# Rikorose/DeepFilterNet

Hardware: AMD Instinct MI355X
Metric: 48 kHz audio frames/sec (hop=480), DeepFilterNet3 enhance() (higher is better)
Workload: dtype f32 (storage and accumulation; GRU projections / recurrences, the fused DF-encoder convolutions and the pointwise halves of the ERB separable convolutions as fp16-split MFMAs: x = hi + lo in f16, hi*hi + hi*lo + lo*hi on v_mfma_f32_16x16x32_f16, ~2^-21 relative; see exact_fp32_ms_per_step); 1 GPU; DeepFilterNet3 (recalled shipped shape, conv_ch=64) enhance(pad=True), batch=256 clips x 10 s @48 kHz per GPU, 1002 STFT frames per clip; batch_per_gpu=256, global_batch=256, parallelism=clips sharded over 1 GPU(s); no collective, inputs_resident_in_hbm=True

## Files before the change

deepfilternet_amd/csrc/dfx_nn_kernels.h:

```cpp
#pragma once

#include "dfx_common.h"

#include <type_traits>

#define DFX_ACT_NONE 0
#define DFX_ACT_RELU 1
#define DFX_ACT_TANH 2
#define DFX_ACT_SIGMOID 3

static __device__ __forceinline__ float dfx_sigmoid(float x) { return 1.f / (1.f + expf(-x)); }
static __device__ __forceinline__ float dfx_act(float v, int act) {
    if (act == DFX_ACT_RELU) return fmaxf(v, 0.f);
    if (act == DFX_ACT_TANH) return tanhf(v);
    if (act == DFX_ACT_SIGMOID) return dfx_sigmoid(v);
    return v;
}

static __device__ __forceinline__ float dfx_row256_scale_split(const float4 (&raw)[16], dfx_h8 (&xh)[8], dfx_h8 (&xl)[8]) {
    float mx = 0.f;
#pragma unroll
    for (int i = 0; i < 16; ++i) mx = fmaxf(mx, fmaxf(fmaxf(fabsf(raw[i].x), fabsf(raw[i].y)), fmaxf(fabsf(raw[i].z), fabsf(raw[i].w))));
    mx = fmaxf(mx, __shfl_xor(mx, 16));
    mx = fmaxf(mx, __shfl_xor(mx, 32));
// ... 3940 lines not shown
    dfx_h8 *wl = reinterpret_cast<dfx_h8 *>(smraw);
    uint16_t *h16 = reinterpret_cast<uint16_t *>(smraw + DFX_GH_SMEM_W);
    float *h32 = reinterpret_cast<float *>(smraw + DFX_GH_SMEM_W);
    static_assert((size_t)2 * DFX_GH_ROWS * DFX_GH_HROW32 * 4 <= (size_t)2 * 2 * DFX_GH_ROWS * DFX_GH_HROW * 2, "the fp32 copy of h fits where the f16 copies live");
    constexpr size_t HB_KSTEP = X32 ? 32 * 4 : 32 * 2, HB_LO = X32 ? 16 : (size_t)DFX_GH_ROWS * HROW * 2;
    const int tid = threadIdx.x, lane = tid & 63, wave = tid >> 6, q = lane >> 4, jl = lane & 15;
    const int64_t b0 = grp * DFX_GH_ROWS;
    const bool valid = b0 + jl < A.B;
    const int64_t brow = valid ? b0 + jl : A.B - 1;
    const dfx_h8 *wg = A.whf + lane;
#define DFX_GH_GIDX(f) (((((size_t)wave * NS + DFX_GH_POS_S(f)) * 8 + DFX_GH_POS_KC(f)) * 3 + DFX_GH_POS_GATE(f)) * 2 * 64)
    dfx_h8 wr[FR][2];
    dfx_static_for<0, NF>([&](auto fc) {
        constexpr int f = decltype(fc)::value;
        if constexpr (SC.cls[f] == 0) {
            wr[SC.idx[f]][0] = wg[DFX_GH_GIDX(f)];
            wr[SC.idx[f]][1] = wg[DFX_GH_GIDX(f) + 64];
            if constexpr (DFX_GH_PIN && !X32) {
                DFX_PIN_AGPR(wr[SC.idx[f]][0]);
                DFX_PIN_AGPR(wr[SC.idx[f]][1]);
            }
        } else if constexpr (SC.cls[f] == 1) {
            wl[((SC.idx[f] * NW + wave) * 2 + 0) * 64 + lane] = wg[DFX_GH_GIDX(f)];
            wl[((SC.idx[f] * NW + wave) * 2 + 1) * 64 + lane] = wg[DFX_GH_GIDX(f) + 64];
        }
    });
    float hp[NS][4];
    float4 bn[NS];
#pragma unroll
    for (int s = 0; s < NS; ++s) {
        const int u0 = UW * wave + 16 * s + 4 * q;
        bn[s] = *reinterpret_cast<const float4 *>(A.bhn + u0);
        float4 h0 = make_float4(0.f, 0.f, 0.f, 0.f);
        if (A.h_in) h0 = *reinterpret_cast<const float4 *>(A.h_in + brow * H + u0);
        hp[s][0] = h0.x, hp[s][1] = h0.y, hp[s][2] = h0.z, hp[s][3] = h0.w;
    }
    auto put_h16 = [&](int buf, int s) {
        if constexpr (X32) {
            *reinterpret_cast<float4 *>(h32 + ((size_t)buf * DFX_GH_ROWS + jl) * DFX_GH_HROW32 + UW * wave + 16 * s + 4 * q) =
                make_float4(hp[s][0], hp[s][1], hp[s][2], hp[s][3]);
            return;
        }
        uint16_t hh[4], hl[4];
#pragma unroll
        for (int r = 0; r < 4; ++r) {
            hh[r] = dfx_f32_to_f16_bits(hp[s][r]);
            hl[r] = dfx_f32_to_f16_bits(hp[s][r] - dfx_f16_bits_to_f32(hh[r]));
        }
        const int col = UW * wave + 16 * s + 4 * q;
        uint16_t *ph = h16 + ((size_t)(buf * 2 + 0) * DFX_GH_ROWS + jl) * HROW + col;
        uint16_t *pl = h16 + ((size_t)(buf * 2 + 1) * DFX_GH_ROWS + jl) * HROW + col;
        *reinterpret_cast<uint2 *>(ph) = make_uint2((uint32_t)hh[0] | ((uint32_t)hh[1] << 16), (uint32_t)hh[2] | ((uint32_t)hh[3] << 16));
        *reinterpret_cast<uint2 *>(pl) = make_uint2((uint32_t)hl[0] | ((uint32_t)hl[1] << 16), (uint32_t)hl[2] | ((uint32_t)hl[3] << 16));
    };
#pragma unroll
    for (int s = 0; s < NS; ++s) put_h16(0, s);
    __syncthreads();
    dfx_h8 ring[D][2];
    dfx_static_for<0, D>([&](auto dc) {
        constexpr int d = decltype(dc)::value;
        ring[d][0] = wg[DFX_GH_GIDX(SC.spos[d])];
        ring[d][1] = wg[DFX_GH_GIDX(SC.spos[d]) + 64];
    });
    const float *gp = A.gi + brow * A.T * (3 * H) + UW * wave + 4 * q;
    float *yp = A.y + brow * A.T * H + UW * wave + 4 * q;
    int cur = 0;
    float4 gv[3][NS];
#pragma unroll
    for (int g = 0; g < 3; ++g)
#pragma unroll
        for (int s = 0; s < NS; ++s) gv[g][s] = make_float4(0.1f, 0.2f, 0.3f, 0.4f);
    DfxWaiter W{Y.spin_limit, Y.err};
    auto wait_gi = [&](int64_t upto) {
        if (tid == 0) W.wait_ge<2>(Y.giprog, Y.pbase + (unsigned int)(upto < A.T ? upto : A.T));
        __syncthreads();
        dfx_xcd_acquire(Y.x);
    };
    if (SEQ) dfx_xcd_register(Y.x);
    const int nchunk = SEQ ? Y.K : 1;
    for (int ck = 0; ck < nchunk; ++ck) {
    const int64_t c0 = SEQ ? (int64_t)Y.tb[ck] : A.t0, c1 = SEQ ? (int64_t)Y.tb[ck + 1] : A.t1;
    if (SEQ) {
        if (tid == 0 && Y.trace) Y.trace[ck * 3 + 0] = wall_clock64();
        if (tid == 0 && !Y.giprog) W.wait_ge<8>(Y.ready, Y.base + (unsigned int)ck + 1u);
        __syncthreads();
        dfx_sync_acquire(false);
        if (Y.giprog && ck == 0) wait_gi(Y.sblk);
        if (tid == 0 && Y.trace) Y.trace[ck * 3 + 1] = wall_clock64();
    }
#pragma unroll
    for (int g = 0; g < 3; ++g)
#pragma unroll
        for (int s = 0; s < NS; ++s)
            if (c1 > c0 && !(DFX_GH_ABLATE & 2)) gv[g][s] = *reinterpret_cast<const float4 *>(gp + c0 * (3 * H) + g * H + 16 * s);
    for (int64_t t = c0; t < c1; ++t) {
        if (SEQ && Y.giprog && ((t + 1) & (Y.sblk - 1)) == 0 && t + 1 < A.T) wait_gi(t + 1 + Y.sblk);
        int zoff = 0;
        DFX_OPAQUE(zoff);
        const dfx_h8 *wst = wg + zoff;
        const int64_t tn = t + 1 < c1 ? t + 1 : t;
        const unsigned char *hb = X32 ? reinterpret_cast<const unsigned char *>(h32 + ((size_t)cur * DFX_GH_ROWS + jl) * DFX_GH_HROW32 + 8 * q)
                                      : reinterpret_cast<const unsigned char *>(h16 + (size_t)(cur * 2) * DFX_GH_ROWS * HROW + (size_t)jl * HROW + 8 * q);
        f32x4 acc[TILES];
#pragma unroll
        for (int i = 0; i < TILES; ++i) acc[i] = f32x4{0.f, 0.f, 0.f, 0.f};
        dfx_h8 bh[2], bl[2];
        bh[0] = *reinterpret_cast<const dfx_h8 *>(hb);
        bl[0] = *reinterpret_cast<const dfx_h8 *>(hb + HB_LO);
        auto gate_unit = [&](int s, int r) {
            const float gr = r == 0 ? gv[0][s].x : r == 1 ? gv[0][s].y : r == 2 ? gv[0][s].z : gv[0][s].w;
            const float gz = r == 0 ? gv[1][s].x : r == 1 ? gv[1][s].y : r == 2 ? gv[1][s].z : gv[1][s].w;
            const float gn = r == 0 ? gv[2][s].x : r == 1 ? gv[2][s].y : r == 2 ? gv[2][s].z : gv[2][s].w;
            const float bb = r == 0 ? bn[s].x : r == 1 ? bn[s].y : r == 2 ? bn[s].z : bn[s].w;
            if (DFX_GH_ABLATE & 8) {
                hp[s][r] = 0.5f * hp[s][r] + 1e-3f * (gr + gz + gn + bb + acc[s][r] + acc[NS + s][r] + acc[2 * NS + s][r]);
                return;
            }
            const float rg = dfx_fast_rcp(1.f + dfx_fast_exp(-(gr + acc[0 * NS + s][r] * A.unscale)));
            const float zg = dfx_fast_rcp(1.f + dfx_fast_exp(-(gz + acc[1 * NS + s][r] * A.unscale)));
            const float pre = gn + rg * (acc[2 * NS + s][r] * A.unscale + bb);
            const float ng = 2.f * dfx_fast_rcp(1.f + dfx_fast_exp(-2.f * pre)) - 1.f;
            hp[s][r] = (1.f - zg) * ng + zg * hp[s][r];
        };
        auto gate_finish = [&](int s) {
            if (!(DFX_GH_ABLATE & 2)) {
#pragma unroll
                for (int g = 0; g < 3; ++g) gv[g][s] = *reinterpret_cast<const float4 *>(gp + tn * (3 * H) + g * H + 16 * s);
            }
            if (valid && !(DFX_GH_ABLATE & 16)) *reinterpret_cast<float4 *>(yp + t * H + 16 * s) = make_float4(hp[s][0], hp[s][1], hp[s][2], hp[s][3]);
            put_h16(cur ^ 1, s);
        };
        dfx_static_for<0, NF / 3>([&](auto gc) {
            constexpr int grp = decltype(gc)::value, f0 = 3 * grp;
            constexpr int kc = DFX_GH_POS_KC(f0), tt0 = DFX_GH_POS_TT(f0);
            if constexpr (tt0 == (DFX_GH_TILES / 6) * 3 && kc + 1 < 8) {
                constexpr int kn = kc + 1;
                bh[kn & 1] = *reinterpret_cast<const dfx_h8 *>(hb + HB_KSTEP * kn);
                bl[kn & 1] = *reinterpret_cast<const dfx_h8 *>(hb + HB_LO + HB_KSTEP * kn);
            }
            dfx_h8 whi[3], wlo[3];
            dfx_static_for<0, 3>([&](auto ic) {
                constexpr int i = decltype(ic)::value, f = f0 + i;
                if constexpr (SC.cls[f] == 0) {
                    whi[i] = wr[SC.idx[f]][0];
                    wlo[i] = wr[SC.idx[f]][1];
                } else if constexpr (SC.cls[f] == 1) {
                    whi[i] = wl[((SC.idx[f] * NW + wave) * 2 + 0) * 64 + lane];
                    wlo[i] = wl[((SC.idx[f] * NW + wave) * 2 + 1) * 64 + lane];
                } else {
                    whi[i] = ring[SC.idx[f] % D][0];
                    wlo[i] = ring[SC.idx[f] % D][1];
                }
            });
            constexpr int ta = DFX_GH_POS_TILE(f0), tb_ = DFX_GH_POS_TILE(f0 + 1), tc = DFX_GH_POS_TILE(f0 + 2);
            if constexpr (X32) {
                const f32x4 b0 = __builtin_bit_cast(f32x4, bh[kc & 1]), b1 = __builtin_bit_cast(f32x4, bl[kc & 1]);
                const f32x4 a0[3] = {__builtin_bit_cast(f32x4, whi[0]), __builtin_bit_cast(f32x4, whi[1]), __builtin_bit_cast(f32x4, whi[2])};
                const f32x4 a1[3] = {__builtin_bit_cast(f32x4, wlo[0]), __builtin_bit_cast(f32x4, wlo[1]), __builtin_bit_cast(f32x4, wlo[2])};
#pragma unroll
                for (int j = 0; j < 4; ++j) {
                    acc[ta] = __builtin_amdgcn_mfma_f32_16x16x4f32(a0[0][j], b0[j], acc[ta], 0, 0, 0);
                    acc[tb_] = __builtin_amdgcn_mfma_f32_16x16x4f32(a0[1][j], b0[j], acc[tb_], 0, 0, 0);
                    acc[tc] = __builtin_amdgcn_mfma_f32_16x16x4f32(a0[2][j], b0[j], acc[tc], 0, 0, 0);
                }
#pragma unroll
                for (int j = 0; j < 4; ++j) {
                    acc[ta] = __builtin_amdgcn_mfma_f32_16x16x4f32(a1[0][j], b1[j], acc[ta], 0, 0, 0);
                    acc[tb_] = __builtin_amdgcn_mfma_f32_16x16x4f32(a1[1][j], b1[j], acc[tb_], 0, 0, 0);
                    acc[tc] = __builtin_amdgcn_mfma_f32_16x16x4f32(a1[2][j], b1[j], acc[tc], 0, 0, 0);
                }
            } else if (!(DFX_GH_ABLATE & 4)) {
                acc[ta] = dfx_mfma_16x16x32_f16(wlo[0], bh[kc & 1], acc[ta]);
                acc[tb_] = dfx_mfma_16x16x32_f16(wlo[1], bh[kc & 1], acc[tb_]);
                acc[tc] = dfx_mfma_16x16x32_f16(wlo[2], bh[kc & 1], acc[tc]);
                acc[ta] = dfx_mfma_16x16x32_f16(whi[0], bl[kc & 1], acc[ta]);
                acc[tb_] = dfx_mfma_16x16x32_f16(whi[1], bl[kc & 1], acc[tb_]);
                acc[tc] = dfx_mfma_16x16x32_f16(whi[2], bl[kc & 1], acc[tc]);
                acc[ta] = dfx_mfma_16x16x32_f16(whi[0], bh[kc & 1], acc[ta]);
                acc[tb_] = dfx_mfma_16x16x32_f16(whi[1], bh[kc & 1], acc[tb_]);
                acc[tc] = dfx_mfma_16x16x32_f16(whi[2], bh[kc & 1], acc[tc]);
            } else {
                acc[ta][0] += (float)whi[0][0] + (float)wlo[0][1] + (float)bh[kc & 1][0] + (float)bl[kc & 1][0];
                acc[tb_][0] += (float)whi[1][0] + (float)wlo[1][1] + (float)bh[kc & 1][0] + (float)bl[kc & 1][0];
                acc[tc][0] += (float)whi[2][0] + (float)wlo[2][1] + (float)bh[kc & 1][0] + (float)bl[kc & 1][0];
            }
            DFX_SCHED_BARRIER();
            dfx_static_for<0, 3>([&](auto ic) {
                constexpr int f = f0 + decltype(ic)::value;
                if constexpr (SC.cls[f] == 2 && !(DFX_GH_ABLATE & 1)) {
                    constexpr int nxt = SC.spos[(SC.idx[f] + D) % FS];
                    ring[SC.idx[f] % D][0] = wst[DFX_GH_GIDX(nxt)];
                    ring[SC.idx[f] % D][1] = wst[DFX_GH_GIDX(nxt) + 64];
                }
            });
            DFX_SCHED_BARRIER();
        });
#pragma unroll
        for (int s = 0; s < NS; ++s) {
#pragma unroll
            for (int r = 0; r < 4; ++r) gate_unit(s, r);
            gate_finish(s);
        }
        const bool ypub = SEQ && Y.yprog && (((t + 1) & (Y.yblk - 1)) == 0 || t + 1 == A.T);
        if (ypub) DFX_VMEM_DRAIN();
        __syncthreads();
        cur ^= 1;
        if (ypub && tid == 0) dfx_xcd_release(Y.x, Y.yprog, Y.pbase + (unsigned int)(t + 1));
    }
    if (SEQ) {
        __builtin_amdgcn_fence(__ATOMIC_RELEASE, "agent");
        __syncthreads();
        if (tid == 0) dfx_sync_raise(Y.done + grp, Y.base + (unsigned int)ck + 1u, false);
        if (tid == 0 && Y.trace) Y.trace[ck * 3 + 2] = wall_clock64();
    }
    }
    if (A.h_out && valid) {
#pragma unroll
        for (int s = 0; s < NS; ++s)
            *reinterpret_cast<float4 *>(A.h_out + brow * H + UW * wave + 16 * s + 4 * q) = make_float4(hp[s][0], hp[s][1], hp[s][2], hp[s][3]);
    }
}
#undef DFX_GH_GIDX

template <bool X32>
static __device__ __forceinline__ void dfx_gru_rec_body(const DfxGhArgs &A) {
    int64_t grp = blockIdx.x;
    if (A.xcd_mask) {
        const int x = dfx_xcc_id();
        if (!((A.xcd_mask >> x) & 1)) return;
        grp = (int64_t)(blockIdx.x >> 3) * __builtin_popcount(A.xcd_mask) + __builtin_popcount(A.xcd_mask & ((1 << x) - 1));
        if (grp * DFX_GH_ROWS >= A.B) return;
    }
    dfx_gru_h3_run<false, X32>(A, grp, DfxGhSync{nullptr, nullptr, 0u, 1, nullptr, nullptr, nullptr, 0});
}
__global__ void __launch_bounds__(DFX_GH_THREADS, DFX_GH_NW / 4) dfx_k_gru_rec_h3(DfxGhArgs A) { dfx_gru_rec_body<false>(A); }
__global__ void __launch_bounds__(DFX_GH_THREADS, DFX_GH_NW / 4) dfx_k_gru_rec_x32(DfxGhArgs A) { dfx_gru_rec_body<true>(A); }

struct DfxGsArgs {
    const float *gi[DFX_GS_MAX_LAYERS];
    float *y[DFX_GS_MAX_LAYERS];
    const dfx_h8 *whf[DFX_GS_MAX_LAYERS];
    const float *bhn[DFX_GS_MAX_LAYERS];
    float unscale[DFX_GS_MAX_LAYERS];
    int64_t B, T;
    int nlayers, groups, K;
    int tb[DFX_GS_MAX_CHUNKS + 1];
    unsigned int *ready;
    unsigned int *done;
    int done_stride;
    unsigned int base;
    unsigned int *err;
    unsigned long long *trace;
    int spin_limit;
    unsigned int *yprog[DFX_GS_MAX_LAYERS] = {};
    unsigned int *giprog[DFX_GS_MAX_LAYERS] = {};
    unsigned int pbase = 0;
    int sblk = 16;
    int yblk[DFX_GS_MAX_LAYERS] = {};
    unsigned int *xtab = nullptr;
    int xstride = 0;
    int xcons_kind[DFX_GS_MAX_LAYERS] = {}, xcons_layer[DFX_GS_MAX_LAYERS] = {};
    unsigned int xtag = 0;
    unsigned int *xstat = nullptr;
    int pair_far = 0;
    unsigned int *psync = nullptr;
};
template <bool X32>
static __device__ __forceinline__ void dfx_gru_seq_body(const DfxGsArgs &S) {
    const int l = (int)(blockIdx.x / (unsigned)S.groups), g = (int)(blockIdx.x % (unsigned)S.groups);
    if (l >= S.nlayers) return;
    DfxGhArgs A;
    A.gi = S.gi[l];
    A.whf = S.whf[l];
    A.bhn = S.bhn[l];
    A.h_in = nullptr;
    A.h_out = nullptr;
    A.y = S.y[l];
    A.B = S.B;
    A.T = S.T;
    A.t0 = 0;
    A.t1 = S.T;
    A.unscale = S.unscale[l];
    A.xcd_mask = 0;
    DfxGhSync Y{S.ready + l, S.done + (size_t)l * S.done_stride, S.base, S.K, S.tb, S.err,
                S.trace ? S.trace + ((size_t)l * S.groups + g) * S.K * 3 : nullptr, S.spin_limit};
    Y.yprog = S.yprog[l] ? S.yprog[l] + g : nullptr;
    Y.giprog = S.giprog[l] ? S.giprog[l] + g : nullptr;
    Y.pbase = S.pbase, Y.sblk = S.sblk, Y.yblk = S.yblk[l] > 0 ? S.yblk[l] : 16;
    if (S.xtab) {
        auto word = [&](int kind, int layer) { return S.xtab + ((size_t)kind * DFX_GS_MAX_LAYERS + layer) * S.xstride + g; };
        Y.x.me = word(0, l);
        Y.x.prod = Y.giprog ? word(1, l) : nullptr;
        Y.x.cons = Y.yprog ? word(S.xcons_kind[l], S.xcons_layer[l]) : nullptr;
        Y.x.tag = S.xtag, Y.x.stat = S.xstat;
    }
    dfx_gru_h3_run<true, X32>(A, g, Y);
}
__global__ void __launch_bounds__(DFX_GH_THREADS, DFX_GH_NW / 4) dfx_k_gru_seq(DfxGsArgs S) { dfx_gru_seq_body<false>(S); }
__global__ void __launch_bounds__(DFX_GH_THREADS, DFX_GH_NW / 4) dfx_k_gru_seq_x32(DfxGsArgs S) { dfx_gru_seq_body<true>(S); }

#include "dfx_gru_pair.h"

#define DFX_PF_MAX 4
struct DfxPfArgs {
    const float *x[DFX_PF_MAX];
    float *gi[DFX_PF_MAX];
    const dfx_h8 *wf[DFX_PF_MAX];
    const float *bias[DFX_PF_MAX];
    float unscale[DFX_PF_MAX];
    const unsigned int *yprog[DFX_PF_MAX];
    unsigned int *giprog[DFX_PF_MAX];
    int64_t B, T;
    int nf, groups;
    unsigned int pbase;
    unsigned int *err;
    int spin_limit;
    const unsigned int *xprod[DFX_PF_MAX] = {};
    unsigned int *xme[DFX_PF_MAX] = {};
    const unsigned int *xcons[DFX_PF_MAX] = {};
    unsigned int xtag = 0;
    unsigned int *xstat = nullptr;
    const unsigned int *xrec = nullptr;
    unsigned int *xclaim = nullptr;
};
static __device__ __forceinline__ DfxXcd dfx_pf_xcd(const DfxPfArgs &A, int f, int g) {
    DfxXcd X;
    if (A.xme[f]) X.me = A.xme[f] + g, X.prod = A.xprod[f] ? A.xprod[f] + g : nullptr, X.cons = A.xcons[f] ? A.xcons[f] + g : nullptr, X.tag = A.xtag, X.stat = A.xstat;
    return X;
}
static __device__ __forceinline__ bool dfx_pf_begin(const DfxPfArgs &A, DfxWaiter &W, int *slot, int &f, int &g) {
    f = (int)(blockIdx.x / (unsigned)A.groups);
    if (f >= A.nf) return false;
    g = dfx_xcd_claim(A.xrec ? (A.xcons[f] ? A.xcons[f] : A.xrec) : nullptr, A.xtag, A.groups,
                      A.xclaim ? A.xclaim + 8 * f : nullptr, (int)(blockIdx.x % (unsigned)A.groups), W, slot);
    dfx_xcd_register(dfx_pf_xcd(A, f, g));
    return true;
}
static __device__ __forceinline__ void dfx_pf_wait_block(const DfxPfArgs &A, DfxWaiter &W, int f, int g, int t1) {
    if (threadIdx.x == 0) W.wait_ge<4>(A.yprog[f] + g, A.pbase + (unsigned int)t1);
    __syncthreads();
    dfx_xcd_acquire(dfx_pf_xcd(A, f, g));
}
static __device__ __forceinline__ void dfx_pf_raise_block(const DfxPfArgs &A, int f, int g, int t1) {
    if (threadIdx.x == 0) dfx_xcd_release(dfx_pf_xcd(A, f, g), A.giprog[f] + g, A.pbase + (unsigned int)t1);
}
__global__ void __launch_bounds__(512, 1) dfx_k_proj_follow(DfxPfArgs A) {
    constexpr int NW = 8, CT = 4, NTH = 64 * NW, SB = 2 * NW, N = 768;
    constexpr int CH8 = 8 * CT * 2 * 64;
    constexpr int PER_T = CH8 / NTH;
    DFX_DYN_SMEM(dfx_h8, ws);
    DfxWaiter W{A.spin_limit, A.err};
    int f, g;
    if (!dfx_pf_begin(A, W, reinterpret_cast<int *>(ws), f, g)) return;
    const int tid = threadIdx.x, lane = tid & 63, wave = tid >> 6, q = lane >> 4, jl = lane & 15;
    constexpr int nchunks = N / (16 * CT);
    const int T = (int)A.T;
    for (int t0 = 0; t0 < T; t0 += SB) {
        const int t1 = t0 + SB < T ? t0 + SB : T;
        int zoff = 0, jz = jl;
        DFX_OPAQUE(zoff);
        DFX_OPAQUE(jz);
        const dfx_h8 *wf = A.wf[f] + zoff;
        const float *bias = A.bias[f] + zoff;
        const int64_t clip = (int64_t)g * 16 + jz;
        const bool okc = clip < A.B;
        const float *xrow = A.x[f] + (okc ? clip : 0) * A.T * 256 + 8 * q;
        float *orow = A.gi[f] + (okc ? clip : 0) * A.T * N;
#pragma unroll
        for (int i = 0; i < PER_T; ++i) ws[i * NTH + tid] = wf[i * NTH + tid];
        dfx_pf_wait_block(A, W, f, g, t1);
        dfx_h8 xh[2][8], xl[2][8];
        float unscale[2];
        int trow[2];
        bool okr[2];
#pragma unroll
        for (int t = 0; t < 2; ++t) {
            trow[t] = t0 + 2 * wave + t;
            okr[t] = okc && trow[t] < t1;
            if (!okr[t]) trow[t] = t0;
            unscale[t] = A.unscale[f] * dfx_row256_split(xrow + trow[t] * 256, okr[t], xh[t], xl[t]);
        }
        for (int c = 0; c < nchunks; ++c) {
            const dfx_h8 *wc = ws + (size_t)(c & 1) * CH8;
            constexpr int HP = PER_T / 2;
            dfx_h8 pre[HP];
            const dfx_h8 *src = wf + (size_t)(c + 1) * CH8;
            dfx_h8 *dst = ws + (size_t)((c + 1) & 1) * CH8;
            if (c + 1 < nchunks) {
#pragma unroll
                for (int i = 0; i < HP; ++i) pre[i] = src[i * NTH + tid];
            }
            f32x4 acc[2][CT];
#pragma unroll
            for (int t = 0; t < 2; ++t)
#pragma unroll
                for (int ct = 0; ct < CT; ++ct) acc[t][ct] = f32x4{0.f, 0.f, 0.f, 0.f};
#pragma unroll
            for (int kc = 0; kc < 8; ++kc) {
                dfx_h8 whi[CT], wlo[CT];
#pragma unroll
                for (int ct = 0; ct < CT; ++ct) {
                    whi[ct] = wc[((kc * CT + ct) * 2 + 0) * 64 + lane];
                    wlo[ct] = wc[((kc * CT + ct) * 2 + 1) * 64 + lane];
                }
#pragma unroll
                for (int ct = 0; ct < CT; ++ct)
#pragma unroll
                    for (int t = 0; t < 2; ++t) acc[t][ct] = dfx_mfma_16x16x32_f16(wlo[ct], xh[t][kc], acc[t][ct]);
#pragma unroll
                for (int ct = 0; ct < CT; ++ct)
#pragma unroll
                    for (int t = 0; t < 2; ++t) acc[t][ct] = dfx_mfma_16x16x32_f16(whi[ct], xl[t][kc], acc[t][ct]);
#pragma unroll
                for (int ct = 0; ct < CT; ++ct)
#pragma unroll
                    for (int t = 0; t < 2; ++t) acc[t][ct] = dfx_mfma_16x16x32_f16(whi[ct], xh[t][kc], acc[t][ct]);
                if (kc == 3 && c + 1 < nchunks) {
#pragma unroll
                    for (int i = 0; i < HP; ++i) dst[i * NTH + tid] = pre[i];
#pragma unroll
                    for (int i = 0; i < HP; ++i) pre[i] = src[(HP + i) * NTH + tid];
                }
            }
#pragma unroll
            for (int ct = 0; ct < CT; ++ct) {
                const int n = c * (16 * CT) + 16 * ct + 4 * q;
                const float4 bz = *reinterpret_cast<const float4 *>(bias + n);
#pragma unroll
                for (int t = 0; t < 2; ++t)
                    if (okr[t])
                        *reinterpret_cast<float4 *>(orow + trow[t] * N + n) =
                            make_float4(acc[t][ct][0] * unscale[t] + bz.x, acc[t][ct][1] * unscale[t] + bz.y, acc[t][ct][2] * unscale[t] + bz.z,
                                        acc[t][ct][3] * unscale[t] + bz.w);
            }
            if (c + 1 < nchunks) {
#pragma unroll
                for (int i = 0; i < HP; ++i) dst[(HP + i) * NTH + tid] = pre[i];
            } else {
                DFX_VMEM_DRAIN();
            }
            __syncthreads();
        }
        dfx_pf_raise_block(A, f, g, t1);
    }
}

__global__ void __launch_bounds__(512, 1) dfx_k_proj_follow_x32(DfxPfArgs A) {
    constexpr int NW = 8, CT = 4, NTH = 64 * NW, SB = 2 * NW, N = 768, K = 256;
    constexpr int CHF = K * 16 * CT;
    constexpr int PER_T = CHF / 4 / NTH;
    constexpr int HP = PER_T / 2;
    DFX_DYN_SMEM(float, wsf);
    DfxWaiter W{A.spin_limit, A.err};
    int f, g;
    if (!dfx_pf_begin(A, W, reinterpret_cast<int *>(wsf), f, g)) return;
    const int tid = threadIdx.x, lane = tid & 63, wave = tid >> 6, q = lane >> 4, jl = lane & 15;
    constexpr int nchunks = N / (16 * CT);
    const int T = (int)A.T;
    const int kt = tid >> 4, n4 = tid & 15;
    const int src_off = kt * N + 4 * n4;
    const int dst_off0 = 4 * kt * 64 + 4 * n4, dst_off1 = 4 * kt * 64 + ((4 * n4) ^ 16);
    auto piece_src = [&](const float *w, int c, int i) -> const f32x4 * {
        return reinterpret_cast<const f32x4 *>(w + src_off + 32 * i * N + 64 * c);
    };
    auto piece_dst = [&](float *buf, int i) -> f32x4 * {
        return reinterpret_cast<f32x4 *>(buf + (((i >> 1) & 1) ? dst_off1 : dst_off0) + (128 * (i & 1) + (i >> 1)) * 64);
    };
    for (int t0 = 0; t0 < T; t0 += SB) {
        const int t1 = t0 + SB < T ? t0 + SB : T;
        int zoff = 0, jz = jl;
        DFX_OPAQUE(zoff);
        DFX_OPAQUE(jz);
        const float *w = reinterpret_cast<const float *>(A.wf[f]) + zoff;
        const float *bias = A.bias[f] + zoff;
        const int64_t clip = (int64_t)g * 16 + jz;
        const bool okc = clip < A.B;
        const float *xrow = A.x[f] + (okc ? clip : 0) * A.T * K + 64 * q;
        float *orow = A.gi[f] + (okc ? clip : 0) * A.T * N;
#pragma unroll
        for (int i = 0; i < PER_T; ++i) *piece_dst(wsf, i) = *piece_src(w, 0, i);
        dfx_pf_wait_block(A, W, f, g, t1);
        float4 xv[2][16];
        int trow[2];
        bool okr[2];
#pragma unroll
        for (int t = 0; t < 2; ++t) {
            trow[t] = t0 + 2 * wave + t;
            okr[t] = okc && trow[t] < t1;
            if (!okr[t]) trow[t] = t0;
            const float4 *p = reinterpret_cast<const float4 *>(xrow + trow[t] * K);
#pragma unroll
            for (int v = 0; v < 16; ++v) xv[t][v] = okr[t] ? p[v] : make_float4(0.f, 0.f, 0.f, 0.f);
        }
        for (int c = 0; c < nchunks; ++c) {
            const float *wc = wsf + (size_t)(c & 1) * CHF + q * 64 + jl;
            float *dstb = wsf + (size_t)((c + 1) & 1) * CHF;
            f32x4 pre[HP];
            if (c + 1 < nchunks) {
#pragma unroll
                for (int i = 0; i < HP; ++i) pre[i] = *piece_src(w, c + 1, i);
            }
            f32x4 acc[2][CT];
#pragma unroll
            for (int t = 0; t < 2; ++t)
#pragma unroll
                for (int ct = 0; ct < CT; ++ct) acc[t][ct] = f32x4{0.f, 0.f, 0.f, 0.f};
            float fa[2][CT];
#pragma unroll
            for (int ct = 0; ct < CT; ++ct) fa[0][ct] = wc[16 * (ct ^ (q & 1))];
            auto ksteps = [&](auto kc) {
                constexpr int ks = decltype(kc)::value;
                if constexpr (ks + 1 < 64) {
#pragma unroll
                    for (int ct = 0; ct < CT; ++ct) fa[(ks + 1) & 1][ct] = wc[(ks + 1) * 256 + 16 * (ct ^ (q & 1))];
                }
#pragma unroll
                for (int t = 0; t < 2; ++t) {
                    const float4 x4 = xv[t][ks >> 2];
                    const float xk = (ks & 3) == 0 ? x4.x : (ks & 3) == 1 ? x4.y : (ks & 3) == 2 ? x4.z : x4.w;
#pragma unroll
                    for (int ct = 0; ct < CT; ++ct) acc[t][ct] = __builtin_amdgcn_mfma_f32_16x16x4f32(fa[ks & 1][ct], xk, acc[t][ct], 0, 0, 0);
                }
                DFX_SCHED_BARRIER();
            };
            dfx_static_for<0, 32>(ksteps);
            if (c + 1 < nchunks) {
#pragma unroll
                for (int i = 0; i < HP; ++i) *piece_dst(dstb, i) = pre[i];
#pragma unroll
                for (int i = 0; i < HP; ++i) pre[i] = *piece_src(w, c + 1, HP + i);
            }
            dfx_static_for<32, 64>(ksteps);
            DFX_MFMA_GUARD();
#pragma unroll
            for (int ct = 0; ct < CT; ++ct) {
                const int n = c * (16 * CT) + 16 * ct + 4 * q;
                const float4 bz = *reinterpret_cast<const float4 *>(bias + n);
#pragma unroll
                for (int t = 0; t < 2; ++t)
                    if (okr[t])
                        *reinterpret_cast<float4 *>(orow + trow[t] * N + n) =
                            make_float4(acc[t][ct][0] + bz.x, acc[t][ct][1] + bz.y, acc[t][ct][2] + bz.z, acc[t][ct][3] + bz.w);
            }
            if (c + 1 < nchunks) {
#pragma unroll
                for (int i = 0; i < HP; ++i) *piece_dst(dstb, HP + i) = pre[i];
            } else {
                DFX_VMEM_DRAIN();
            }
            __syncthreads();
        }
        dfx_pf_raise_block(A, f, g, t1);
    }
}
```

deepfilternet_amd/csrc/env_hip/dfx_env.h:

```cpp
#pragma once

#include <hip/hip_runtime.h>

#include <cstdint>
#include <cstdio>
#include <cstdlib>
#include <cstring>
#include <utility>

typedef float f32x4 __attribute__((ext_vector_type(4)));
typedef float f32x2 __attribute__((ext_vector_type(2)));
typedef float f32x16 __attribute__((ext_vector_type(16)));

#define DFX_DYN_SMEM(T, name)                                                        \
    extern __shared__ __attribute__((aligned(16))) unsigned char dfx_dyn_smem_raw[]; \
    T *name = reinterpret_cast<T *>(dfx_dyn_smem_raw)

template <typename... KArgs, typename... Args>
static inline void dfx_launch(void (*kernel)(KArgs...), dim3 grid, dim3 block, size_t shmem, hipStream_t stream,
                              Args &&...args) {
    hipLaunchKernelGGL(kernel, grid, block, shmem, stream, static_cast<KArgs>(args)...);
}

static inline int dfx_env_num_cus() {
    static int n = -1;
    if (n < 0) {
        int dev = 0;
        hipDeviceProp_t prop;
        if (hipGetDevice(&dev) == hipSuccess && hipGetDeviceProperties(&prop, dev) == hipSuccess)
            n = prop.multiProcessorCount;
        else
            n = 256;
    }
    return n;
}
static inline int dfx_env_num_xcds() { return dfx_env_num_cus() / 32; }
static inline bool dfx_env_is_emulator() { return false; }
static __device__ __forceinline__ int dfx_wave_uniform(int v) { return __builtin_amdgcn_readfirstlane(v); }
#define DFX_NT_LOAD(p) __builtin_nontemporal_load(p)
#define DFX_NT_STORE(v, p) __builtin_nontemporal_store(v, p)
static __device__ __forceinline__ int dfx_xcc_id() { return (int)__builtin_amdgcn_s_getreg((3 << 11) | 20); }
static inline hipError_t dfx_env_set_max_dyn_smem(const void *func, size_t bytes) {
    return hipFuncSetAttribute(func, hipFuncAttributeMaxDynamicSharedMemorySize, (int)bytes);
}

static inline hipError_t dfx_env_err_words_alloc(unsigned int **host, unsigned int **dev, size_t bytes) {
    void *h = nullptr, *d = nullptr;
    hipError_t e = hipHostMalloc(&h, bytes, hipHostMallocMapped | hipHostMallocCoherent);
    if (e != hipSuccess) return e;
    memset(h, 0, bytes);
    e = hipHostGetDevicePointer(&d, h, 0);
    if (e != hipSuccess) {
        (void)hipHostFree(h);
        return e;
    }
    *host = static_cast<unsigned int *>(h), *dev = static_cast<unsigned int *>(d);
    return hipSuccess;
}
static inline void dfx_env_err_words_free(unsigned int *host) {
    if (host) (void)hipHostFree(host);
}
static __device__ __forceinline__ void dfx_raise(unsigned int *word) { __hip_atomic_store(word, 1u, __ATOMIC_RELAXED, __HIP_MEMORY_SCOPE_SYSTEM); }

typedef _Float16 dfx_h8 __attribute__((ext_vector_type(8)));
static __device__ __host__ __forceinline__ uint16_t dfx_f32_to_f16_bits(float x) {
    const _Float16 h = (_Float16)x;
    uint16_t b;
    __builtin_memcpy(&b, &h, 2);
    return b;
}
static __device__ __host__ __forceinline__ float dfx_f16_bits_to_f32(uint16_t b) {
    _Float16 h;
    __builtin_memcpy(&h, &b, 2);
    return (float)h;
}
typedef _Float16 dfx_h2v __attribute__((ext_vector_type(2)));
typedef float dfx_f2v __attribute__((ext_vector_type(2)));
static __device__ __forceinline__ void dfx_split8(const float *x, dfx_h8 &hi, dfx_h8 &lo) {
#pragma unroll
    for (int i = 0; i < 8; i += 2) {
        const dfx_f2v v = {x[i], x[i + 1]};
        const dfx_h2v h = __builtin_convertvector(v, dfx_h2v);
        const dfx_f2v r = v - __builtin_convertvector(h, dfx_f2v);
        const dfx_h2v l = __builtin_convertvector(r, dfx_h2v);
        hi[i] = h[0], hi[i + 1] = h[1];
        lo[i] = l[0], lo[i + 1] = l[1];
    }
}
#define DFX_H3_LIMIT 6.0e4f
static __device__ __forceinline__ void dfx_split8_g(const float *x, dfx_h8 &hi, dfx_h8 &lo, float &amax) {
#ifndef DFX_NO_H3_GUARD
    amax = fmaxf(amax, fmaxf(fmaxf(fmaxf(fabsf(x[0]), fabsf(x[1])), fmaxf(fabsf(x[2]), fabsf(x[3]))),
                             fmaxf(fmaxf(fabsf(x[4]), fabsf(x[5])), fmaxf(fabsf(x[6]), fabsf(x[7])))));
#endif
    dfx_split8(x, hi, lo);
}
static __device__ __forceinline__ f32x4 dfx_mfma_16x16x32_f16(dfx_h8 a, dfx_h8 b, f32x4 c) {
#ifdef DFX_MFMA_K16
    typedef _Float16 dfx_h4v __attribute__((ext_vector_type(4)));
    const dfx_h4v a0 = {a[0], a[1], a[2], a[3]}, a1 = {a[4], a[5], a[6], a[7]}, b0 = {b[0], b[1], b[2], b[3]}, b1 = {b[4], b[5], b[6], b[7]};
    c = __builtin_amdgcn_mfma_f32_16x16x16f16(a0, b0, c, 0, 0, 0);
    return __builtin_amdgcn_mfma_f32_16x16x16f16(a1, b1, c, 0, 0, 0);
#else
    return __builtin_amdgcn_mfma_f32_16x16x32_f16(a, b, c, 0, 0, 0);
#endif
}

static __device__ __forceinline__ float dfx_lane_gather4(float v, unsigned byte_addr) {
    return __builtin_bit_cast(float, __builtin_amdgcn_ds_bpermute((int)byte_addr, __builtin_bit_cast(int, v)));
}
#define DFX_MUL24(a, b) __mul24((a), (b))
#define DFX_OPAQUE(x) asm volatile("" : "+v"(x))
#define DFX_ASSUME(c) __builtin_assume(c)
#define DFX_PIN_AGPR(x) asm volatile("" : "+a"(x))
#define DFX_SCHED_BARRIER() __builtin_amdgcn_sched_barrier(0)
#define DFX_MFMA_GUARD()                         \
    do {                                         \
        __builtin_amdgcn_sched_barrier(0);       \
        asm volatile("s_nop 7");                 \
        __builtin_amdgcn_sched_barrier(0);       \
    } while (0)
#define DFX_VMEM_DRAIN() asm volatile("s_waitcnt vmcnt(0)" ::: "memory")
#define DFX_L1_INV() asm volatile("buffer_inv sc0" ::: "memory")
#define DFX_SCHED_GROUP(mask, n) __builtin_amdgcn_sched_group_barrier(mask, n, 0)
#ifdef DFX_WAVE_SYNC_WAIT
#define DFX_WAVE_SYNC()                                          \
    do {                                                         \
        __builtin_amdgcn_fence(__ATOMIC_RELEASE, "wavefront");   \
        asm volatile("s_waitcnt lgkmcnt(0)" ::: "memory");       \
        __builtin_amdgcn_wave_barrier();                         \
        __builtin_amdgcn_fence(__ATOMIC_ACQUIRE, "wavefront");   \
    } while (0)
#else
#define DFX_WAVE_SYNC()                                          \
    do {                                                         \
        __builtin_amdgcn_fence(__ATOMIC_RELEASE, "wavefront");   \
        __builtin_amdgcn_wave_barrier();                         \
        __builtin_amdgcn_fence(__ATOMIC_ACQUIRE, "wavefront");   \
    } while (0)
#endif

static __device__ __forceinline__ float dfx_fast_exp(float x) { return __expf(x); }
#ifndef DFX_RCP_RN
static __device__ __forceinline__ float dfx_fast_rcp(float x) { return __builtin_amdgcn_rcpf(x); }
#else
static __device__ __forceinline__ float dfx_fast_rcp(float x) { return __frcp_rn(x); }
#endif
```

Before: 24.85 million frames/s.

## Stream proj_follow weights via global_load_lds and overlap stores with MFMA halves

Reworks the follow-projection kernel so the weight chunks are copied straight from global memory into LDS with global_load_lds. This replaces the old path that staged them through registers and then wrote them to LDS. Each 64-column chunk is split into two halves whose output stores and bias loads are interleaved with the other half's MFMAs, and the next chunk's pieces are requested during the first half. The aim is to cut register pressure and VMEM/LDS store stalls and to hide output writes behind compute. In exchange the schedule gets more complex, and optional trace/ablation instrumentation is added behind macros.

```diff
diff --git a/deepfilternet_amd/csrc/dfx_nn_kernels.h b/deepfilternet_amd/csrc/dfx_nn_kernels.h
--- a/deepfilternet_amd/csrc/dfx_nn_kernels.h
+++ b/deepfilternet_amd/csrc/dfx_nn_kernels.h
@@ -4266,6 +4266,9 @@
 #include "dfx_gru_pair.h"
 
 #define DFX_PF_MAX 4
+#ifndef DFX_PF_TRACE
+#define DFX_PF_TRACE 0
+#endif
 struct DfxPfArgs {
     const float *x[DFX_PF_MAX];
     float *gi[DFX_PF_MAX];
@@ -4286,6 +4289,9 @@
     unsigned int *xstat = nullptr;
     const unsigned int *xrec = nullptr;
     unsigned int *xclaim = nullptr;
+#if DFX_PF_TRACE
+    unsigned long long *trace = nullptr;
+#endif
 };
 static __device__ __forceinline__ DfxXcd dfx_pf_xcd(const DfxPfArgs &A, int f, int g) {
     DfxXcd X;
@@ -4308,6 +4314,24 @@
 static __device__ __forceinline__ void dfx_pf_raise_block(const DfxPfArgs &A, int f, int g, int t1) {
     if (threadIdx.x == 0) dfx_xcd_release(dfx_pf_xcd(A, f, g), A.giprog[f] + g, A.pbase + (unsigned int)t1);
 }
+#ifndef DFX_HAS_GLDS16
+static __device__ __forceinline__ void dfx_glds16(const dfx_h8 *src, dfx_h8 *lds_wave) { lds_wave[threadIdx.x & 63] = *src; }
+#endif
+#ifndef DFX_PF_ABLATE
+#define DFX_PF_ABLATE 0
+#endif
+#define DFX_PF_NPH 8
+#if DFX_PF_TRACE
+#define DFX_PF_STAMP(i)                                                                 \
+    do {                                                                                \
+        unsigned long long now_;                                                        \
+        asm volatile("s_memtime %0\n\ts_waitcnt lgkmcnt(0)" : "=s"(now_)::"memory");    \
+        tk[i] += now_ - tlast;                                                          \
+        tlast = now_;                                                                   \
+    } while (0)
+#else
+#define DFX_PF_STAMP(i) do { } while (0)
+#endif
 __global__ void __launch_bounds__(512, 1) dfx_k_proj_follow(DfxPfArgs A) {
     constexpr int NW = 8, CT = 4, NTH = 64 * NW, SB = 2 * NW, N = 768;
     constexpr int CH8 = 8 * CT * 2 * 64;
@@ -4317,8 +4341,13 @@
     int f, g;
     if (!dfx_pf_begin(A, W, reinterpret_cast<int *>(ws), f, g)) return;
     const int tid = threadIdx.x, lane = tid & 63, wave = tid >> 6, q = lane >> 4, jl = lane & 15;
+    const int wave_u = dfx_wave_uniform(wave);
     constexpr int nchunks = N / (16 * CT);
     const int T = (int)A.T;
+#if DFX_PF_TRACE
+    unsigned long long tk[DFX_PF_NPH] = {}, tlast;
+    asm volatile("s_memtime %0\n\ts_waitcnt lgkmcnt(0)" : "=s"(tlast)::"memory");
+#endif
     for (int t0 = 0; t0 < T; t0 += SB) {
         const int t1 = t0 + SB < T ? t0 + SB : T;
         int zoff = 0, jz = jl;
@@ -4330,9 +4359,39 @@
         const bool okc = clip < A.B;
         const float *xrow = A.x[f] + (okc ? clip : 0) * A.T * 256 + 8 * q;
         float *orow = A.gi[f] + (okc ? clip : 0) * A.T * N;
-#pragma unroll
-        for (int i = 0; i < PER_T; ++i) ws[i * NTH + tid] = wf[i * NTH + tid];
+        auto request_piece = [&](int c, int i) {
+            if (DFX_PF_ABLATE & 2) return;
+            dfx_glds16(wf + (size_t)c * CH8 + i * NTH + tid, ws + (size_t)(c & 1) * CH8 + i * NTH + wave_u * 64);
+        };
+        auto request = [&](int c) {
+#pragma unroll
+            for (int i = 0; i < PER_T; ++i) request_piece(c, i);
+        };
+        auto bias_rows = [&](int c, int h, float4 (&bz)[2]) {
+#pragma unroll
+            for (int j = 0; j < 2; ++j) bz[j] = *reinterpret_cast<const float4 *>(bias + c * (16 * CT) + 16 * (2 * h + j) + 4 * q);
+        };
+        auto bias_ready = [&](float4 (&bz)[2]) {
+#pragma unroll
+            for (int j = 0; j < 2; ++j) {
+                DFX_OPAQUE(bz[j].x);
+                DFX_OPAQUE(bz[j].y);
+                DFX_OPAQUE(bz[j].z);
+                DFX_OPAQUE(bz[j].w);
+            }
+        };
+        static_assert(nchunks % 2 == 0 && nchunks >= 2, "chunk 0 of every block goes to buffer 0");
+        request(0);
+        float4 bzA[2], bzB[2];
+        bias_rows(0, 0, bzA);
+        bias_rows(0, 1, bzB);
+        DFX_PF_STAMP(0);
+        DFX_VMEM_DRAIN();
+        bias_ready(bzA);
+        bias_ready(bzB);
         dfx_pf_wait_block(A, W, f, g, t1);
+        DFX_PF_STAMP(1);
+        request(1);
         dfx_h8 xh[2][8], xl[2][8];
         float unscale[2];
         int trow[2];
@@ -4344,69 +4403,87 @@
             if (!okr[t]) trow[t] = t0;
             unscale[t] = A.unscale[f] * dfx_row256_split(xrow + trow[t] * 256, okr[t], xh[t], xl[t]);
         }
+        DFX_PF_STAMP(2);
+        f32x4 accA[2][2], accB[2][2];
+        auto store_tile = [&](int c, int h, int j, const f32x4 (&acc)[2][2], const float4 (&bz)[2]) {
+            const int n = c * (16 * CT) + 16 * (2 * h + j) + 4 * q;
+#pragma unroll
+            for (int t = 0; t < 2; ++t)
+                if (okr[t] && (!(DFX_PF_ABLATE & 1) || acc[t][j][0] == 1.2345e-30f))
+                    *reinterpret_cast<float4 *>(orow + trow[t] * N + n) =
+                        make_float4(acc[t][j][0] * unscale[t] + bz[j].x, acc[t][j][1] * unscale[t] + bz[j].y, acc[t][j][2] * unscale[t] + bz[j].z,
+                                    acc[t][j][3] * unscale[t] + bz[j].w);
+        };
+        auto half = [&](int c, int h, f32x4 (&acc)[2][2], auto &&under) {
+            const dfx_h8 *wc = ws + (size_t)(c & 1) * CH8;
+#pragma unroll
+            for (int t = 0; t < 2; ++t)
+#pragma unroll
+                for (int j = 0; j < 2; ++j) acc[t][j] = f32x4{0.f, 0.f, 0.f, 0.f};
+            dfx_static_for<0, 8>([&](auto kk) {
+                constexpr int kc = decltype(kk)::value;
+                dfx_h8 whi[2], wlo[2];
+#pragma unroll
+                for (int j = 0; j < 2; ++j) {
+                    whi[j] = wc[((kc * CT + 2 * h + j) * 2 + 0) * 64 + lane];
+                    wlo[j] = wc[((kc * CT + 2 * h + j) * 2 + 1) * 64 + lane];
+                }
+#pragma unroll
+                for (int j = 0; j < 2; ++j)
+#pragma unroll
+                    for (int t = 0; t < 2; ++t) acc[t][j] = dfx_mfma_16x16x32_f16(wlo[j], xh[t][kc], acc[t][j]);
+#pragma unroll
+                for (int j = 0; j < 2; ++j)
+#pragma unroll
+                    for (int t = 0; t < 2; ++t) acc[t][j] = dfx_mfma_16x16x32_f16(whi[j], xl[t][kc], acc[t][j]);
+#pragma unroll
+                for (int j = 0; j < 2; ++j)
+#pragma unroll
+                    for (int t = 0; t < 2; ++t) acc[t][j] = dfx_mfma_16x16x32_f16(whi[j], xh[t][kc], acc[t][j]);
+                under(kk);
+            });
+        };
         for (int c = 0; c < nchunks; ++c) {
-            const dfx_h8 *wc = ws + (size_t)(c & 1) * CH8;
-            constexpr int HP = PER_T / 2;
-            dfx_h8 pre[HP];
-            const dfx_h8 *src = wf + (size_t)(c + 1) * CH8;
-            dfx_h8 *dst = ws + (size_t)((c + 1) & 1) * CH8;
-            if (c + 1 < nchunks) {
-#pragma unroll
-                for (int i = 0; i < HP; ++i) pre[i] = src[i * NTH + tid];
-            }
-            f32x4 acc[2][CT];
-#pragma unroll
-            for (int t = 0; t < 2; ++t)
-#pragma unroll
-                for (int ct = 0; ct < CT; ++ct) acc[t][ct] = f32x4{0.f, 0.f, 0.f, 0.f};
-#pragma unroll
-            for (int kc = 0; kc < 8; ++kc) {
-                dfx_h8 whi[CT], wlo[CT];
-#pragma unroll
-                for (int ct = 0; ct < CT; ++ct) {
-                    whi[ct] = wc[((kc * CT + ct) * 2 + 0) * 64 + lane];
-                    wlo[ct] = wc[((kc * CT + ct) * 2 + 1) * 64 + lane];
-                }
-#pragma unroll
-                for (int ct = 0; ct < CT; ++ct)
-#pragma unroll
-                    for (int t = 0; t < 2; ++t) acc[t][ct] = dfx_mfma_16x16x32_f16(wlo[ct], xh[t][kc], acc[t][ct]);
-#pragma unroll
-                for (int ct = 0; ct < CT; ++ct)
-#pragma unroll
-                    for (int t = 0; t < 2; ++t) acc[t][ct] = dfx_mfma_16x16x32_f16(whi[ct], xl[t][kc], acc[t][ct]);
-#pragma unroll
-                for (int ct = 0; ct < CT; ++ct)
-#pragma unroll
-                    for (int t = 0; t < 2; ++t) acc[t][ct] = dfx_mfma_16x16x32_f16(whi[ct], xh[t][kc], acc[t][ct]);
-                if (kc == 3 && c + 1 < nchunks) {
-#pragma unroll
-                    for (int i = 0; i < HP; ++i) dst[i * NTH + tid] = pre[i];
-#pragma unroll
-                    for (int i = 0; i < HP; ++i) pre[i] = src[(HP + i) * NTH + tid];
-                }
-            }
-#pragma unroll
-            for (int ct = 0; ct < CT; ++ct) {
-                const int n = c * (16 * CT) + 16 * ct + 4 * q;
-                const float4 bz = *reinterpret_cast<const float4 *>(bias + n);
-#pragma unroll
-                for (int t = 0; t < 2; ++t)
-                    if (okr[t])
-                        *reinterpret_cast<float4 *>(orow + trow[t] * N + n) =
-                            make_float4(acc[t][ct][0] * unscale[t] + bz.x, acc[t][ct][1] * unscale[t] + bz.y, acc[t][ct][2] * unscale[t] + bz.z,
-                                        acc[t][ct][3] * unscale[t] + bz.w);
-            }
-            if (c + 1 < nchunks) {
-#pragma unroll
-                for (int i = 0; i < HP; ++i) dst[(HP + i) * NTH + tid] = pre[i];
-            } else {
-                DFX_VMEM_DRAIN();
-            }
+            half(c, 0, accA, [&](auto kk) {
+                constexpr int kc = decltype(kk)::value;
+                if (c > 0) {
+                    if (kc < 4 && c + 1 < nchunks) {
+                        request_piece(c + 1, 2 * kc);
+                        request_piece(c + 1, 2 * kc + 1);
+                    }
+                    if (kc == 1) store_tile(c - 1, 1, 0, accB, bzB);
+                    if (kc == 3) store_tile(c - 1, 1, 1, accB, bzB);
+                }
+                if (kc == 4) bias_rows(c, 1, bzB);
+            });
+            DFX_PF_STAMP(3);
+            half(c, 1, accB, [&](auto kk) {
+                constexpr int kc = decltype(kk)::value;
+                if (kc == 0) store_tile(c, 0, 0, accA, bzA);
+                if (kc == 2) store_tile(c, 0, 1, accA, bzA);
+                if (kc == 3 && c + 1 < nchunks) bias_rows(c + 1, 0, bzA);
+            });
+            DFX_PF_STAMP(6);
+            if (c + 1 == nchunks) {
+                bias_ready(bzB);
+                DFX_MFMA_GUARD();
+                store_tile(c, 1, 0, accB, bzB);
+                store_tile(c, 1, 1, accB, bzB);
+            }
+            DFX_VMEM_DRAIN();
+            bias_ready(bzA);
+            bias_ready(bzB);
+            DFX_PF_STAMP(4);
             __syncthreads();
+            DFX_PF_STAMP(5);
         }
         dfx_pf_raise_block(A, f, g, t1);
-    }
+        DFX_PF_STAMP(7);
+    }
+#if DFX_PF_TRACE
+    if (tid == 0 && A.trace)
+        for (int i = 0; i < DFX_PF_NPH; ++i) A.trace[(size_t)blockIdx.x * DFX_PF_NPH + i] = tk[i];
+#endif
 }
 
 __global__ void __launch_bounds__(512, 1) dfx_k_proj_follow_x32(DfxPfArgs A) {
diff --git a/deepfilternet_amd/csrc/env_hip/dfx_env.h b/deepfilternet_amd/csrc/env_hip/dfx_env.h
--- a/deepfilternet_amd/csrc/env_hip/dfx_env.h
+++ b/deepfilternet_amd/csrc/env_hip/dfx_env.h
@@ -123,6 +123,10 @@
 #define DFX_VMEM_DRAIN() asm volatile("s_waitcnt vmcnt(0)" ::: "memory")
 #define DFX_L1_INV() asm volatile("buffer_inv sc0" ::: "memory")
 #define DFX_SCHED_GROUP(mask, n) __builtin_amdgcn_sched_group_barrier(mask, n, 0)
+#define DFX_HAS_GLDS16 1
+static __device__ __forceinline__ void dfx_glds16(const dfx_h8 *src, dfx_h8 *lds_wave) {
+    __builtin_amdgcn_global_load_lds((const __attribute__((address_space(1))) void *)src, (__attribute__((address_space(3))) void *)lds_wave, 16, 0, 0);
+}
 #ifdef DFX_WAVE_SYNC_WAIT
 #define DFX_WAVE_SYNC()                                          \
     do {                                                         \
```

New measurement: 24.86 million frames/s (median of 5 runs). Within noise of the previous version (+0.0%).
